# vadimkantorov/convasr

Hardware: NVIDIA B200
Metric: audio_seconds_per_second (higher is better)
Workload: dtype bf16

## Files before the change

### convasr_b200/csrc/common.cuh

```cuda
#pragma once
#include <cuda_runtime.h>
#include <cuda_bf16.h>
#include <cuda_fp16.h>
#include <cuda.h>
#include <stdint.h>
#include <math.h>

namespace cab {

void set_last_error(const char* fmt, ...);

#define CAB_CHECK_ARG(cond, ...)                                  \
    do {                                                          \
        if (!(cond)) {                                            \
            ::cab::set_last_error(__VA_ARGS__);                   \
            return -1;                                            \
        }                                                         \
    } while (0)

#define CAB_CHECK_CUDA(expr)                                                              \
    do {                                                                                  \
        cudaError_t _e = (expr);                                                          \
        if (_e != cudaSuccess) {                                                          \
            ::cab::set_last_error("%s failed: %s (%s:%d)", #expr, cudaGetErrorString(_e), \
// ... 81 lines not shown
        : "=r"(ok)
        : "r"(smem_u32(bar)), "r"(parity)
        : "memory");
    return ok != 0;
}
#ifndef CAB_MBAR_SPIN_LIMIT
#define CAB_MBAR_SPIN_LIMIT (1u << 28)
#endif
__device__ __forceinline__ void mbar_wait(uint64_t* bar, uint32_t parity) {
    uint32_t spins = 0;
    while (!mbar_try_wait(bar, parity)) {
        if (++spins > CAB_MBAR_SPIN_LIMIT) __trap();
    }
}

__device__ __forceinline__ void tma_prefetch_desc(const CUtensorMap* m) {
    asm volatile("prefetch.tensormap [%0];" ::"l"(reinterpret_cast<uint64_t>(m)) : "memory");
}
__device__ __forceinline__ void tma_load_3d(void* smem_dst, const CUtensorMap* m, uint64_t* bar,
                                            int c0, int c1, int c2) {
    asm volatile(
        "cp.async.bulk.tensor.3d.shared::cluster.global.tile.mbarrier::complete_tx::bytes "
        "[%0], [%1, {%3, %4, %5}], [%2];"
        ::"r"(smem_u32(smem_dst)), "l"(reinterpret_cast<uint64_t>(m)), "r"(smem_u32(bar)),
        "r"(c0), "r"(c1), "r"(c2)
        : "memory");
}

__device__ __forceinline__ void tma_load_4d(void* smem_dst, const CUtensorMap* m, uint64_t* bar,
                                            int c0, int c1, int c2, int c3) {
// ... 32 lines not shown
        "setp.ne.b32 p, %4, 0;\n\t"
        "tcgen05.mma.cta_group::1.kind::f16 [%0], %1, %2, %3, p;\n\t"
        "}\n"
        ::"r"(tmem_d), "l"(desc_a), "l"(desc_b), "r"(idesc), "r"(accumulate)
        : "memory");
}
__device__ __forceinline__ void umma_e4m3(uint32_t tmem_d, uint64_t desc_a, uint64_t desc_b,
                                          uint32_t idesc, uint32_t accumulate) {
    asm volatile(
        "{\n\t"
        ".reg .pred p;\n\t"
        "setp.ne.b32 p, %4, 0;\n\t"
        "tcgen05.mma.cta_group::1.kind::f8f6f4 [%0], %1, %2, %3, p;\n\t"
        "}\n"
        ::"r"(tmem_d), "l"(desc_a), "l"(desc_b), "r"(idesc), "r"(accumulate)
        : "memory");
}
__device__ __forceinline__ void umma_commit(uint64_t* bar) {
    asm volatile("tcgen05.commit.cta_group::1.mbarrier::arrive::one.shared::cluster.b64 [%0];" ::"r"(
                     smem_u32(bar))
                 : "memory");
}
__device__ __forceinline__ void tmem_ld_32x32(uint32_t taddr, uint32_t (&v)[32]) {
    asm volatile(
        "tcgen05.ld.sync.aligned.32x32b.x32.b32 "
        "{%0, %1, %2, %3, %4, %5, %6, %7, %8, %9, %10, %11, %12, %13, %14, %15, "
        "%16, %17, %18, %19, %20, %21, %22, %23, %24, %25, %26, %27, %28, %29, %30, %31}, [%32];"
        : "=r"(v[0]), "=r"(v[1]), "=r"(v[2]), "=r"(v[3]), "=r"(v[4]), "=r"(v[5]), "=r"(v[6]),
          "=r"(v[7]), "=r"(v[8]), "=r"(v[9]), "=r"(v[10]), "=r"(v[11]), "=r"(v[12]), "=r"(v[13]),
          "=r"(v[14]), "=r"(v[15]), "=r"(v[16]), "=r"(v[17]), "=r"(v[18]), "=r"(v[19]),
// ... 53 lines not shown
```

### convasr_b200/csrc/conv_gemm.cu

```cuda
#include "common.cuh"
#include "../../include/convasr_b200.h"
#include <mutex>
#include <atomic>

namespace cab {

constexpr int kBlockM = 128;
constexpr int kBlockK = 64;
constexpr int kStages = 4;
constexpr int kMaxBlockN = 256;
constexpr int kATileBytes = kBlockM * kBlockK * 2;
constexpr int kBTileBytes = kMaxBlockN * kBlockK * 2;
constexpr int kStageBytes = kATileBytes + kBTileBytes;
constexpr int kAccStages = 2;
constexpr int kTmemCols = 512;
constexpr int kNumThreads = 256;
constexpr int kEpiCols = 32;
constexpr int kEpiTileBytes = kBlockM * kEpiCols * 2;
constexpr int kOffStageOut = kStages * kStageBytes;
constexpr int kOffBias = kOffStageOut + 4 * kEpiTileBytes;
constexpr int kOffBars = kOffBias + kMaxBlockN * 4;
constexpr int kSmemBytes = kOffBars + 1024  + 256 ;
static_assert(kSmemBytes <= 232448, "exceeds the 227 KB dynamic shared memory limit");

struct SrcDev {
    int a_ch_off, w_ch_off, n_chunks, taps, dil, pad_left;
};

struct alignas(64) ConvParams {
    CUtensorMap amap[CAB_MAX_CONV_SOURCES];
    CUtensorMap wmap[CAB_MAX_CONV_SOURCES];
    CUtensorMap omap_hi, omap_lo;
    SrcDev src[CAB_MAX_CONV_SOURCES];
    int n_src;
    int B, T_out, C_out, block_n;
    int mtiles_per_b, n_ntiles, n_tiles;
    int epilogue, act;
    float act_a, act_b;
    const float* bias;
    const float* xlen;
    __nv_bfloat16* out_hi;
    __nv_bfloat16* out_lo;
    int out_T_rows, out_ld;
    float* logits;
    float* log_probs;
    int* argmax;
    double* stats;
    float* lse;
    int mtile_major;
    const float* skip_frac;
    int skip_T, skip_margin;
// ... 3 lines not shown
    double* bnr_partials;
    int bnr_C, bnr_act;
    float bnr_a, bnr_b;
    const float* alpha;
    float out_inv;
};

__device__ __forceinline__ int live_mtiles(const ConvParams& p, int b) {
    if (p.skip_frac == nullptr) return p.mtiles_per_b;
    const int rows = min(p.T_out, frac_len(__ldg(p.skip_frac + b), p.skip_T) + p.skip_margin);
    return rows <= 0 ? 0 : (rows + 127) / 128;
}
#define CAB_NEXT_UNIT()                                                        \
    int am, nt;                                                                \
    if (p.mtile_major) {                                                       \
        if (nt_next == 0) u += gridDim.x;                                      \
        am = u;                                                                \
        nt = nt_next;                                                          \
        nt_next = nt_next + 1 == p.n_ntiles ? 0 : nt_next + 1;                 \
    } else {                                                                   \
        u += gridDim.x;                                                        \
        nt = u % p.n_ntiles;                                                   \
        am = u / p.n_ntiles;                                                   \
    }
struct TileCursor {
    int b, base, end;
    __device__ __forceinline__ void init(const ConvParams& p) { b = 0; base = 0; end = live_mtiles(p, 0); }
    __device__ __forceinline__ bool seek(const ConvParams& p, int am) {
        while (am >= end) {
            if (++b >= p.B) return false;
            base = end;
            end += live_mtiles(p, b);
        }
        return true;
    }
};

__device__ __forceinline__ float apply_act(float x, int act, float a, float b) {
    switch (act) {
        case CAB_ACT_RELU: return fmaxf(x, 0.f);
        case CAB_ACT_HARDTANH: return fminf(fmaxf(x, a), b);
        case CAB_ACT_LEAKY_RELU: return x > 0.f ? x : x * a;
        default: return x;
    }
}

__device__ __forceinline__ void tma_store_3d(const CUtensorMap* m, const void* smem_src, int c0, int c1, int c2) {
    asm volatile("cp.async.bulk.tensor.3d.global.shared::cta.bulk_group [%0, {%2, %3, %4}], [%1];" ::"l"(
                     reinterpret_cast<uint64_t>(m)),
                 "r"(smem_u32(smem_src)), "r"(c0), "r"(c1), "r"(c2)
// ... 92 lines not shown
    const int cq = c >> 3, cb = (c & 7) << 1;
    float s = 0.f, q = 0.f;
#pragma unroll 8
    for (int r = rg * 32; r < r_end; ++r) {
        const int off = r * 64 + ((cq ^ ((r >> 1) & 3)) << 4) + cb;
        float x = __uint_as_float((uint32_t)(*reinterpret_cast<const uint16_t*>(st_h + off)) << 16);
        if (LO) x += __uint_as_float((uint32_t)(*reinterpret_cast<const uint16_t*>(st_l + off)) << 16);
        s += x;
        q = fmaf(x, x, q);
    }
    s_out = s;
    q_out = q;
}

template <bool FP8>
__global__ void __launch_bounds__(kNumThreads, 1)
conv1d_umma_kernel(const __grid_constant__ ConvParams p) {
    constexpr int kChunk = FP8 ? 2 * kBlockK : kBlockK;
    extern __shared__ uint8_t smem_raw[];
    uint8_t* smem = reinterpret_cast<uint8_t*>((reinterpret_cast<uintptr_t>(smem_raw) + 1023) &
                                               ~uintptr_t(1023));
    uint64_t* full_bar = reinterpret_cast<uint64_t*>(smem + kOffBars);
    float* s_bias = reinterpret_cast<float*>(smem + kOffBias);
    uint64_t* empty_bar = full_bar + kStages;
    uint64_t* tmem_full = empty_bar + kStages;
    uint64_t* tmem_empty = tmem_full + kAccStages;
    uint32_t* tmem_ptr = reinterpret_cast<uint32_t*>(tmem_empty + kAccStages);
    uint64_t* ybar = tmem_empty + kAccStages + 1;

    const int warp = threadIdx.x >> 5;
    const int lane = threadIdx.x & 31;

    if (warp == 0 && lane == 0) {
        for (int s = 0; s < p.n_src; ++s) {
            tma_prefetch_desc(&p.amap[s]);
            tma_prefetch_desc(&p.wmap[s]);
        }
        if (p.epilogue == CAB_EPI_LOGITS_ROWS) tma_prefetch_desc(&p.omap_hi);
        if (p.epilogue == CAB_EPI_ACT_BF16) {
            tma_prefetch_desc(&p.omap_hi);
            if (p.out_lo != nullptr) tma_prefetch_desc(&p.omap_lo);
            if (p.bnr_partials != nullptr) tma_prefetch_desc(&p.ymap);
        }
    }
    if (warp == 1 && lane == 0) {
        for (int i = 0; i < kStages; ++i) {
            mbar_init(&full_bar[i], 1);
            mbar_init(&empty_bar[i], 1);
        }
        for (int i = 0; i < kAccStages; ++i) {
            mbar_init(&tmem_full[i], 1);
            mbar_init(&tmem_empty[i], 4);
        }
        mbar_init(&ybar[0], 1);
        mbar_init(&ybar[1], 1);
        mbar_fence_init();
    }
    if (warp == 2) {
        tmem_alloc(tmem_ptr, kTmemCols);
        tmem_relinquish();
    }
    tc_fence_before();
    __syncthreads();
    tc_fence_after();
    const uint32_t tmem_base = *tmem_ptr;

    const int block_n = p.block_n;
    const uint32_t stage_tx_bytes = kATileBytes + block_n * kBlockK * 2;

    if (warp == 0) {
        if (lane == 0) {
            int stage = 0;
            uint32_t phase = 0;
            TileCursor cur;
            cur.init(p);
            int u = (int)blockIdx.x - (int)gridDim.x, nt_next = 0;
            for (;;) {
                CAB_NEXT_UNIT()
                if (!cur.seek(p, am)) break;
                const int b = cur.b;
                const int t0 = (am - cur.base) * kBlockM;
                const int n0 = nt * block_n;
                for (int s = 0; s < p.n_src; ++s) {
                    const SrcDev sd = p.src[s];
                    for (int tap = 0; tap < sd.taps; ++tap) {
                        const int trow = t0 + tap * sd.dil - sd.pad_left;
                        for (int ch = 0; ch < sd.n_chunks; ++ch) {
                            mbar_wait(&empty_bar[stage], phase ^ 1);
                            uint8_t* a_dst = smem + stage * kStageBytes;
                            uint8_t* b_dst = a_dst + kATileBytes;
                            mbar_expect_tx(&full_bar[stage], stage_tx_bytes);
                            tma_load_3d(a_dst, &p.amap[s], &full_bar[stage],
                                        sd.a_ch_off + ch * kChunk, trow, b);
                            tma_load_3d(b_dst, &p.wmap[s], &full_bar[stage],
                                        sd.w_ch_off + ch * kChunk, n0, tap);
                            if (++stage == kStages) { stage = 0; phase ^= 1; }
                        }
                    }
                }
            }
        }
    } else if (warp == 1) {
        if (lane == 0) {
            const uint32_t idesc = FP8 ? umma_idesc_e4m3(kBlockM, block_n) : umma_idesc_bf16(kBlockM, block_n);
            int stage = 0;
            uint32_t phase = 0;
            int acc = 0;
            uint32_t acc_phase = 0;
            TileCursor cur;
            cur.init(p);
            int u = (int)blockIdx.x - (int)gridDim.x, nt_next = 0;
            for (;;) {
                CAB_NEXT_UNIT()
                (void)nt;
                if (!cur.seek(p, am)) break;
                mbar_wait(&tmem_empty[acc], acc_phase ^ 1);
                tc_fence_after();
                const uint32_t d_tmem = tmem_base + acc * kMaxBlockN;
                uint32_t accumulate = 0;
                for (int s = 0; s < p.n_src; ++s) {
                    const int ksteps = p.src[s].taps * p.src[s].n_chunks;
                    for (int ks = 0; ks < ksteps; ++ks) {
                        mbar_wait(&full_bar[stage], phase);
                        tc_fence_after();
                        const uint32_t a_addr = smem_u32(smem + stage * kStageBytes);
                        const uint32_t b_addr = a_addr + kATileBytes;
                        const uint64_t a_desc = umma_desc_sw128(a_addr);
                        const uint64_t b_desc = umma_desc_sw128(b_addr);
#pragma unroll
                        for (int k = 0; k < kBlockK / 16; ++k) {
                            if (FP8) umma_e4m3(d_tmem, a_desc + 2 * k, b_desc + 2 * k, idesc, accumulate);
                            else umma_bf16(d_tmem, a_desc + 2 * k, b_desc + 2 * k, idesc, accumulate);
                            accumulate = 1;
                        }
                        umma_commit(&empty_bar[stage]);
                        if (++stage == kStages) { stage = 0; phase ^= 1; }
                    }
                }
                umma_commit(&tmem_full[acc]);
                if (++acc == kAccStages) { acc = 0; acc_phase ^= 1; }
            }
        }
    } else if (warp >= 4) {
        const int q = warp & 3;
        const int row = q * 32 + lane;
        int acc = 0;
        uint32_t acc_phase = 0;
        uint32_t epi_chunks = 0;
        TileCursor cur;
        cur.init(p);
        float run_m = -INFINITY, run_s = 0.f;
        int run_i = 0;
        uint32_t yphase = 0;
        const bool fold = p.bnr_partials != nullptr;
        int u = (int)blockIdx.x - (int)gridDim.x, nt_next = 0;
        for (;;) {
            CAB_NEXT_UNIT()
            if (!cur.seek(p, am)) break;
            const int b = cur.b;
            const int t0 = (am - cur.base) * kBlockM;
            const int n0 = nt * block_n;
            const int t = t0 + row;
            const bool row_ok = t < p.T_out;

            const uint32_t taddr = tmem_base + acc * kMaxBlockN + (uint32_t(q * 32) << 16);
            if (p.epilogue != CAB_EPI_ACT_BF16) {
                mbar_wait(&tmem_full[acc], acc_phase);
                tc_fence_after();
            }

            if (p.epilogue == CAB_EPI_ACT_BF16) {
                int len = p.T_out;
                if (p.xlen != nullptr) len = frac_len(__ldg(p.xlen + b), p.T_out);
                const bool keep = t < len;
                const int et = threadIdx.x - 128;
                const bool has_lo = p.out_lo != nullptr;
                uint8_t* const ystage = smem + kOffStageOut + 2 * kEpiTileBytes;
                int bnr_rows = 0;
                if (fold) {
                    if (et == 0) {
                        const int ybuf = epi_chunks & 1;
                        mbar_expect_tx(&ybar[ybuf], kEpiTileBytes);
                        tma_load_3d(ystage + ybuf * kEpiTileBytes, &p.ymap, &ybar[ybuf], n0, t0, b);
                    }
                    int blen = p.T_out;
                    if (p.bnr_xlen != nullptr) blen = min(blen, frac_len(__ldg(p.bnr_xlen + b), p.T_out));
                    bnr_rows = min(max(blen - t0, 0), kBlockM);
                }
                epi_bar(1);
                float* const s_alpha = reinterpret_cast<float*>(smem + kOffStageOut + 2 * kEpiTileBytes);
                for (int i = et; i < block_n; i += 128) {
                    const int n = n0 + i;
                    s_bias[i] = (p.bias != nullptr && n < p.C_out) ? __ldg(p.bias + n) : 0.f;
                    if (FP8) s_alpha[i] = n < p.C_out ? __ldg(p.alpha + n) : 0.f;
                }
                epi_bar(1);
                mbar_wait(&tmem_full[acc], acc_phase);
                tc_fence_after();
                uint8_t* stage = smem + kOffStageOut;
                for (int c0 = 0; c0 < block_n; c0 += kEpiCols) {
                    if (n0 + c0 >= p.C_out) break;
                    uint32_t v[32];
                    tmem_ld_32x32(taddr + c0, v);
                    tmem_ld_wait();
                    if (c0 + kEpiCols >= block_n || n0 + c0 + kEpiCols >= p.C_out) {
                        tc_fence_before();
                        __syncwarp();
                        if (lane == 0) mbar_arrive(&tmem_empty[acc]);
                    }
                    const int buf = epi_chunks & 1;
                    uint8_t* st_hi = stage + buf * kEpiTileBytes;
                    uint8_t* st_lo = stage + (2 + buf) * kEpiTileBytes;
                    if (et == 0) bulk_wait_read<1>();
                    float bnr_sc = 0.f, bnr_sh = 0.f;
                    const int bnr_col = n0 + c0 + (et & 31);
                    if (fold && bnr_col < p.bnr_C) {
                        bnr_sc = __ldg(p.bnr_ss + bnr_col);
                        bnr_sh = __ldg(p.bnr_ss + p.bnr_C + bnr_col);
                    }
                    epi_bar(2);
                    if (fold && et == 0 && c0 + kEpiCols < block_n && n0 + c0 + kEpiCols < p.C_out) {
                        const int ynext = (epi_chunks + 1) & 1;
                        mbar_expect_tx(&ybar[ynext], kEpiTileBytes);
// ... 2 lines not shown
                    const float* sb = s_bias + c0;
#define CAB_EPI_CALL(ACT)                                                                          \
    if (FP8) epi_chunk_e4m3<ACT>(v, sb, s_alpha + c0, p.act_a, p.act_b, keep, p.out_inv, row, st_hi); \
    else if (has_lo) epi_chunk<ACT, true>(v, sb, p.act_a, p.act_b, keep, row, st_hi, st_lo);       \
    else epi_chunk<ACT, false>(v, sb, p.act_a, p.act_b, keep, row, st_hi, st_lo);
                    switch (p.act) {
                        case CAB_ACT_RELU: CAB_EPI_CALL(CAB_ACT_RELU) break;
                        case CAB_ACT_HARDTANH: CAB_EPI_CALL(CAB_ACT_HARDTANH) break;
                        case CAB_ACT_LEAKY_RELU: CAB_EPI_CALL(CAB_ACT_LEAKY_RELU) break;
                        default: CAB_EPI_CALL(CAB_ACT_NONE) break;
                    }
#undef CAB_EPI_CALL
                    fence_async_smem();
                    epi_bar(3);
                    if (et == 0) {
                        tma_store_3d(&p.omap_hi, st_hi, n0 + c0, t0, b);
                        if (has_lo) tma_store_3d(&p.omap_lo, st_lo, n0 + c0, t0, b);
                        bulk_commit();
                    }
                    if (p.stats != nullptr) {
                        float cs, cq;
                        const int srows = min(max(p.T_out - t0, 0), kBlockM);
                        if (has_lo) stats_column_pass<true>(st_hi, st_lo, et, srows, cs, cq);
                        else stats_column_pass<false>(st_hi, st_lo, et, srows, cs, cq);
                        const int col = n0 + c0 + (et & 31);
                        if (col < p.C_out && srows > (et >> 5) * 32) {
                            atomicAdd(p.stats + col, (double)cs);
                            atomicAdd(p.stats + p.C_out + col, (double)cq);
                        }
                    }
                    if (fold) {
                        mbar_wait(&ybar[buf], (yphase >> buf) & 1u);
                        yphase ^= 1u << buf;
                        const uint8_t* st_y = ystage + buf * kEpiTileBytes;
                        float cs, cq;
                        switch (p.bnr_act) {
                            case CAB_ACT_RELU: bnr_column_pass<CAB_ACT_RELU>(st_hi, st_y, et, bnr_rows, bnr_sc, bnr_sh, p.bnr_a, p.bnr_b, cs, cq); break;
// ... 18 lines not shown
                for (int i = et; i < block_n; i += 128) {
                    const int n = n0 + i;
                    s_bias[i] = (p.bias != nullptr && n < C) ? __ldg(p.bias + n) : 0.f;
                }
                epi_bar(1);
                if (nt == 0) { run_m = -INFINITY; run_s = 0.f; run_i = 0; }
                uint8_t* stage = smem + kOffStageOut;
                for (int c0 = 0; c0 < block_n; c0 += 32) {
                    if (n0 + c0 >= C) break;
                    uint32_t v[32];
                    tmem_ld_32x32(taddr + c0, v);
                    tmem_ld_wait();
                    if (c0 + 32 >= block_n || n0 + c0 + 32 >= C) {
                        tc_fence_before();
                        __syncwarp();
                        if (lane == 0) mbar_arrive(&tmem_empty[acc]);
                    }
                    float x[32];
                    float cm = -INFINITY;
                    int ci = 0;
#pragma unroll
                    for (int j = 0; j < 32; ++j) {
                        const bool in = n0 + c0 + j < C;
                        if (FP8) x[j] = fmaf(__uint_as_float(v[j]), in ? __ldg(p.alpha + n0 + c0 + j) : 0.f, s_bias[c0 + j]);
                        else x[j] = __uint_as_float(v[j]) + s_bias[c0 + j];
                        if (in && x[j] > cm) { cm = x[j]; ci = n0 + c0 + j; }
                    }
                    if (cm > run_m) {
                        run_s *= __expf(run_m - cm);
                        run_m = cm;
                        run_i = ci;
                    }
                    float cs = 0.f;
#pragma unroll
                    for (int j = 0; j < 32; ++j) cs += (n0 + c0 + j < C) ? __expf(x[j] - run_m) : 0.f;
                    run_s += cs;
                    const int buf = epi_chunks & 1;
                    uint8_t* st = stage + buf * (2 * kEpiTileBytes);
                    if (et == 0) bulk_wait_read<1>();
                    epi_bar(2);
#pragma unroll
                    for (int q4 = 0; q4 < 8; ++q4)
                        *reinterpret_cast<float4*>(st + row * 128 + ((q4 ^ (row & 7)) << 4)) = make_float4(x[4 * q4], x[4 * q4 + 1], x[4 * q4 + 2], x[4 * q4 + 3]);
                    fence_async_smem();
                    epi_bar(3);
                    if (et == 0) {
                        tma_store_3d(&p.omap_hi, st, n0 + c0, t0, b);
                        bulk_commit();
                    }
                    ++epi_chunks;
                }
                if (nt == p.n_ntiles - 1 && row_ok) {
                    if (p.lse) p.lse[size_t(b) * p.T_out + t] = run_m + logf(run_s);
                    if (p.argmax) p.argmax[size_t(b) * p.T_out + t] = run_i;
                }
                if (++acc == kAccStages) { acc = 0; acc_phase ^= 1; }
                continue;
            } else if (p.epilogue == CAB_EPI_LOGSOFTMAX) {
                const int C = p.C_out;
                float vmax = -INFINITY;
                int imax = 0;
                for (int c0 = 0; c0 < C; c0 += 16) {
// ... 50 lines not shown
                    tmem_ld_wait();
                    if (row_ok) {
#pragma unroll
                        for (int j = 0; j < 16; ++j) {
                            const int c = n0 + c0 + j;
                            if (c < C) {
                                float x = (FP8 ? __uint_as_float(v[j]) * __ldg(p.alpha + c) : __uint_as_float(v[j])) + (p.bias ? __ldg(p.bias + c) : 0.f);
                                p.logits[(size_t(b) * C + c) * p.T_out + t] = apply_act(x, p.act, p.act_a, p.act_b);
                            }
                        }
                    }
                }
            }
            tc_fence_before();
            __syncwarp();
            if (lane == 0) mbar_arrive(&tmem_empty[acc]);
            if (++acc == kAccStages) { acc = 0; acc_phase ^= 1; }
        }
        if (p.skip_frac != nullptr && p.epilogue == CAB_EPI_ACT_BF16) {
            const int et = threadIdx.x - 128;
            const bool has_lo = p.out_lo != nullptr;
            uint8_t* stage = smem + kOffStageOut;
            int b = 0, base = 0, end = p.mtiles_per_b - live_mtiles(p, 0);
            for (int z = blockIdx.x;; z += gridDim.x) {
                const int nt = z % p.n_ntiles;
                const int sm = z / p.n_ntiles;
                bool done = false;
                while (sm >= end) {
                    if (++b >= p.B) { done = true; break; }
                    base = end;
                    end += p.mtiles_per_b - live_mtiles(p, b);
                }
                if (done) break;
                const int t0 = (live_mtiles(p, b) + (sm - base)) * kBlockM;
                const int n0 = nt * block_n;
                for (int c0 = 0; c0 < block_n; c0 += kEpiCols) {
                    if (n0 + c0 >= p.C_out) break;
                    const int buf = epi_chunks & 1;
                    uint8_t* st_hi = stage + buf * kEpiTileBytes;
                    uint8_t* st_lo = stage + (2 + buf) * kEpiTileBytes;
                    if (et == 0) bulk_wait_read<1>();
                    epi_bar(2);
                    uint4* zh = reinterpret_cast<uint4*>(st_hi + row * (FP8 ? 32 : 64));
                    uint4* zl = reinterpret_cast<uint4*>(st_lo + row * 64);
#pragma unroll
                    for (int qd = 0; qd < (FP8 ? 2 : 4); ++qd) {
                        zh[qd] = make_uint4(0, 0, 0, 0);
                        if (has_lo) zl[qd] = make_uint4(0, 0, 0, 0);
                    }
                    fence_async_smem();
                    epi_bar(3);
                    if (et == 0) {
                        tma_store_3d(&p.omap_hi, st_hi, n0 + c0, t0, b);
                        if (has_lo) tma_store_3d(&p.omap_lo, st_lo, n0 + c0, t0, b);
                        bulk_commit();
                    }
                    ++epi_chunks;
                }
            }
        }
        if (threadIdx.x == 128) bulk_wait_all();
    }

    tc_fence_before();
    __syncthreads();
    if (warp == 2) {
        tc_fence_after();
        tmem_dealloc(tmem_base, kTmemCols);
    }
}

typedef CUresult (*EncodeTiledFn)(CUtensorMap*, CUtensorMapDataType, cuuint32_t, void*,
                                  const cuuint64_t*, const cuuint64_t*, const cuuint32_t*,
                                  const cuuint32_t*, CUtensorMapInterleave, CUtensorMapSwizzle,
                                  CUtensorMapL2promotion, CUtensorMapFloatOOBfill);

static EncodeTiledFn get_encode_fn() {
    static EncodeTiledFn fn = nullptr;
    static std::once_flag once;
    std::call_once(once, [] {
        void* ptr = nullptr;
        cudaDriverEntryPointQueryResult qres;
        if (cudaGetDriverEntryPoint("cuTensorMapEncodeTiled", &ptr, cudaEnableDefault, &qres) ==
// ... 14 lines not shown
    cuuint32_t box[3] = {box0, box1, 1};
    cuuint32_t estr[3] = {1, 1, 1};
    CUresult r = enc(map, elem_bytes == 1 ? CU_TENSOR_MAP_DATA_TYPE_UINT8 : CU_TENSOR_MAP_DATA_TYPE_BFLOAT16, 3, const_cast<void*>(base), dims,
                     strides, box, estr, CU_TENSOR_MAP_INTERLEAVE_NONE,
                     swizzle, CU_TENSOR_MAP_L2_PROMOTION_L2_256B,
                     CU_TENSOR_MAP_FLOAT_OOB_FILL_NONE);
    CAB_CHECK_ARG(r == CUDA_SUCCESS,
                  "cuTensorMapEncodeTiled failed (%d): base=%p dims=%llu,%llu,%llu pitch=%llu,%llu "
                  "box=%u,%u",
                  (int)r, base, (unsigned long long)d0, (unsigned long long)d1,
                  (unsigned long long)d2, (unsigned long long)pitch1_elems,
                  (unsigned long long)pitch2_elems, box0, box1);
    return 0;
}

static int pick_block_n(int C_out, int epilogue, long long m_tiles, int num_sms) {
    if (epilogue == CAB_EPI_LOGSOFTMAX) return ((C_out + 15) / 16) * 16;
    int best_bn = 0;
    double best_cost = 0.0;
    const int min_tiles = (C_out + kMaxBlockN - 1) / kMaxBlockN;
    for (int n_tiles = min_tiles; n_tiles <= min_tiles * 8; ++n_tiles) {
        int bn = (C_out + n_tiles - 1) / n_tiles;
        bn = ((bn + 31) / 32) * 32;
        if (bn < 64 && n_tiles > min_tiles) break;
        const long long tiles = m_tiles * ((C_out + bn - 1) / bn);
        const double cost = (double)((tiles + num_sms - 1) / num_sms) * (bn + 96);
        if (best_bn == 0 || cost < best_cost * 0.98) { best_bn = bn; best_cost = cost; }
    }
    return best_bn;
}

extern std::atomic<int64_t> g_launch_count;

}

using namespace cab;

template <bool FP8>
static int conv1d_launch(const cab_conv_source_t* srcs, int n_src, const cab_conv_epilogue_t* ep, const float* alpha,
                         float out_inv, cudaStream_t stream) {
    constexpr int kChunk = FP8 ? 2 * kBlockK : kBlockK;
    constexpr int kElem = FP8 ? 1 : 2;
    CAB_CHECK_ARG(srcs && ep, "null sources/epilogue");
    CAB_CHECK_ARG(n_src >= 1 && n_src <= CAB_MAX_CONV_SOURCES, "n_sources=%d out of [1,%d]", n_src,
                  CAB_MAX_CONV_SOURCES);
    CAB_CHECK_ARG(ep->B > 0 && ep->T_out > 0 && ep->C_out > 0, "bad output shape B=%d T=%d C=%d",
                  ep->B, ep->T_out, ep->C_out);

    static thread_local ConvParams p;
    p.n_src = n_src;
    p.B = ep->B;
    p.T_out = ep->T_out;
    p.C_out = ep->C_out;
    static int sms_for_tiling = 0;
    if (sms_for_tiling == 0) {
        int dev = 0;
        cudaGetDevice(&dev);
        cudaDeviceGetAttribute(&sms_for_tiling, cudaDevAttrMultiProcessorCount, dev);
        if (sms_for_tiling <= 0) sms_for_tiling = 148;
    }
    int bn = ep->block_n > 0 ? ep->block_n : pick_block_n(ep->C_out, ep->epilogue, (long long)ep->B * ((ep->T_out + kBlockM - 1) / kBlockM), sms_for_tiling);
    CAB_CHECK_ARG(bn % 16 == 0 && bn >= 16 && bn <= kMaxBlockN, "block_n=%d must be a multiple of 16 in [16,256]", bn);
    if (ep->epilogue == CAB_EPI_ACT_BF16) {
        CAB_CHECK_ARG(bn % 32 == 0, "block_n=%d must be a multiple of 32 for the bf16 epilogue", bn);
        CAB_CHECK_ARG(ep->C_out % 32 == 0, "C_out=%d must be a multiple of 32 (pad on the host)", ep->C_out);
        CAB_CHECK_ARG(ep->out_hi != nullptr, "out_hi is null");
        CAB_CHECK_ARG(ep->out_ld_ch >= ep->C_out && ep->out_ld_ch % 8 == 0, "bad out_ld_ch=%d", ep->out_ld_ch);
        CAB_CHECK_ARG(ep->out_T_rows >= ep->T_out, "out_T_rows=%d < T_out=%d", ep->out_T_rows, ep->T_out);
        CAB_CHECK_ARG((reinterpret_cast<uintptr_t>(ep->out_hi) & 15) == 0, "out_hi must be 16-byte aligned");
    } else if (ep->epilogue == CAB_EPI_LOGSOFTMAX) {
        CAB_CHECK_ARG(ep->C_out <= kMaxBlockN, "log_softmax epilogue supports at most %d classes (got %d)", kMaxBlockN, ep->C_out);
        CAB_CHECK_ARG(bn >= ep->C_out, "block_n=%d must cover all %d classes", bn, ep->C_out);
    } else if (ep->epilogue == CAB_EPI_LOGITS_F32) {
        CAB_CHECK_ARG(ep->logits != nullptr, "logits is null");
    } else if (ep->epilogue == CAB_EPI_LOGITS_ROWS) {
        CAB_CHECK_ARG(ep->logits != nullptr, "logits is null");
        CAB_CHECK_ARG(bn % 32 == 0, "block_n=%d must be a multiple of 32 for the row-major logits epilogue", bn);
        CAB_CHECK_ARG(ep->out_ld_ch >= ep->C_out && ep->out_ld_ch % 4 == 0 && (reinterpret_cast<uintptr_t>(ep->logits) & 15) == 0, "row-major logits need a 16-byte aligned base and a row pitch that is a multiple of 4 floats (got %d)", ep->out_ld_ch);
        CAB_CHECK_ARG(ep->act == CAB_ACT_NONE, "the row-major logits epilogue applies no activation");
    } else {
        CAB_CHECK_ARG(false, "unknown epilogue %d", ep->epilogue);
    }
    p.block_n = bn;
    p.mtiles_per_b = (ep->T_out + kBlockM - 1) / kBlockM;
    p.n_ntiles = (ep->C_out + bn - 1) / bn;
    p.n_tiles = p.B * p.mtiles_per_b * p.n_ntiles;
    p.epilogue = ep->epilogue;
    p.act = ep->act;
    p.act_a = ep->act_a;
    p.act_b = ep->act_b;
    p.bias = ep->bias;
    p.xlen = ep->xlen_frac;
    p.out_hi = static_cast<__nv_bfloat16*>(ep->out_hi);
    p.out_lo = static_cast<__nv_bfloat16*>(ep->out_lo);
    p.out_T_rows = ep->out_T_rows;
    p.out_ld = ep->out_ld_ch;
    p.logits = ep->logits;
    p.log_probs = ep->log_probs;
    p.argmax = ep->argmax;
    p.stats = ep->epilogue == CAB_EPI_ACT_BF16 ? ep->stats : nullptr;
    p.lse = ep->epilogue == CAB_EPI_LOGITS_ROWS ? ep->log_probs : nullptr;
// ... 56 lines not shown
    }

    for (int s = 0; s < n_src; ++s) {
        const cab_conv_source_t& c = srcs[s];
        CAB_CHECK_ARG(c.act && c.wgt, "source %d: null pointer", s);
        CAB_CHECK_ARG(c.C_in > 0 && c.C_in % kChunk == 0, "source %d: C_in=%d must be a multiple of %d", s, c.C_in, kChunk);
        CAB_CHECK_ARG(c.ch_off >= 0 && c.ch_off + c.C_in <= c.ld_ch && c.ld_ch % (16 / kElem) == 0, "source %d: bad channel window off=%d C_in=%d ld=%d", s, c.ch_off, c.C_in, c.ld_ch);
        CAB_CHECK_ARG(c.w_ch_off >= 0 && c.w_ch_off + c.C_in <= c.w_ld_ch && c.w_ld_ch % (16 / kElem) == 0, "source %d: bad weight channel window", s);
        CAB_CHECK_ARG(c.taps >= 1 && c.dilation >= 1, "source %d: taps=%d dilation=%d", s, c.taps, c.dilation);
        CAB_CHECK_ARG(c.T_in >= 1 && c.T_rows >= c.T_in, "source %d: T_in=%d T_rows=%d", s, c.T_in, c.T_rows);
        CAB_CHECK_ARG((reinterpret_cast<uintptr_t>(c.act) & 15) == 0 && (reinterpret_cast<uintptr_t>(c.wgt) & 15) == 0, "source %d: pointers must be 16-byte aligned", s);
        int rc = encode_map_3d(&p.amap[s], c.act, (uint64_t)c.ld_ch, (uint64_t)c.T_in, (uint64_t)ep->B,
                               (uint64_t)c.ld_ch, (uint64_t)c.T_rows * c.ld_ch, kChunk, kBlockM, CU_TENSOR_MAP_SWIZZLE_128B, kElem);
        if (rc) return rc;
        rc = encode_map_3d(&p.wmap[s], c.wgt, (uint64_t)c.w_ld_ch, (uint64_t)c.w_rows, (uint64_t)c.taps,
                           (uint64_t)c.w_ld_ch, (uint64_t)c.w_rows * c.w_ld_ch, kChunk, (uint32_t)bn, CU_TENSOR_MAP_SWIZZLE_128B, kElem);
        if (rc) return rc;
        p.src[s].a_ch_off = c.ch_off;
        p.src[s].w_ch_off = c.w_ch_off;
        p.src[s].n_chunks = c.C_in / kChunk;
        p.src[s].taps = c.taps;
        p.src[s].dil = c.dilation;
        p.src[s].pad_left = c.pad_left;
    }

    static int num_sms = 0;
    static std::once_flag once;
    static cudaError_t attr_err = cudaSuccess;
    std::call_once(once, [] {
        int dev = 0;
        cudaGetDevice(&dev);
        cudaDeviceGetAttribute(&num_sms, cudaDevAttrMultiProcessorCount, dev);
        attr_err = cudaFuncSetAttribute(conv1d_umma_kernel<FP8>, cudaFuncAttributeMaxDynamicSharedMemorySize, kSmemBytes);
    });
    CAB_CHECK_ARG(attr_err == cudaSuccess, "cudaFuncSetAttribute(smem=%d) failed: %s", kSmemBytes, cudaGetErrorString(attr_err));
    CAB_CHECK_ARG(num_sms > 0, "no CUDA device");
    int grid = p.n_tiles < num_sms ? p.n_tiles : num_sms;
    if (p.mtile_major) grid = p.B * p.mtiles_per_b < num_sms ? p.B * p.mtiles_per_b : num_sms;
    conv1d_umma_kernel<FP8><<<grid, kNumThreads, kSmemBytes, stream>>>(p);
    CAB_CHECK_LAUNCH();
    g_launch_count.fetch_add(1, std::memory_order_relaxed);
    return 0;
}

extern "C" int cab_conv1d_fused(const cab_conv_source_t* srcs, int n_src,
                                const cab_conv_epilogue_t* ep, cab_stream_t stream) {
    return conv1d_launch<false>(srcs, n_src, ep, nullptr, 1.f, static_cast<cudaStream_t>(stream));
}

extern "C" int cab_conv1d_fused_fp8(const cab_conv_source_t* srcs, int n_src, const cab_conv_epilogue_t* ep,
                                    const float* alpha, float out_scale_inv, cab_stream_t stream) {
    return conv1d_launch<true>(srcs, n_src, ep, alpha, out_scale_inv, static_cast<cudaStream_t>(stream));
}
// ... 1 lines not shown
```

### convasr_b200/csrc/ctc.cu

```cuda
#include "common.cuh"
#include "../../include/convasr_b200.h"
#include <atomic>
#include <float.h>
#include <cuda_fp16.h>

namespace cab {
extern std::atomic<int64_t> g_launch_count;

constexpr int kCtcMaxPer = 4;

__device__ __forceinline__ float lse3(float a, float b, float c) {
    const float m = fmaxf(a, fmaxf(b, c));
    if (m == -INFINITY) return -INFINITY;
    return logf(expf(a - m) + expf(b - m) + expf(c - m)) + m;
}
__device__ __forceinline__ float lse2(float a, float b) {
    const float m = fmaxf(a, b);
    if (m == -INFINITY) return -INFINITY;
    return logf(expf(a - m) + expf(b - m)) + m;
}

constexpr int kCtcPrefetch = 8;

__device__ __forceinline__ float lse3_fast(float a, float b, float c) {
// ... 366 lines not shown
            if (t > 0) {
                s -= (int)bp[(size_t)t * S_max + s];
                if (s < 0) s = 0;
            }
        }
    }
}

constexpr int kAlignClusterMax = 16;
constexpr int kAlignGroupsPer = 2;
constexpr int kAlignCtaStates = 4 * kAlignGroupsPer * 1024;
constexpr int kAlignLongMaxL = (kAlignClusterMax * kAlignCtaStates - 1) / 2;

__device__ __forceinline__ void cluster_arrive() { asm volatile("barrier.cluster.arrive.release.aligned;" ::: "memory"); }
__device__ __forceinline__ void cluster_wait() { asm volatile("barrier.cluster.wait.acquire.aligned;" ::: "memory"); }
__device__ __forceinline__ uint32_t cluster_ctarank() {
    uint32_t r;
    asm volatile("mov.u32 %0, %%cluster_ctarank;" : "=r"(r));
    return r;
}
__device__ __forceinline__ uint32_t cluster_nctarank() {
    uint32_t r;
    asm volatile("mov.u32 %0, %%cluster_nctarank;" : "=r"(r));
    return r;
}
__device__ __forceinline__ float* cluster_map(float* p, uint32_t rank) {
    uint64_t out;
    asm volatile("mapa.u64 %0, %1, %2;" : "=l"(out) : "l"(reinterpret_cast<uint64_t>(p)), "r"(rank));
    return reinterpret_cast<float*>(out);
}

template <bool HALF>
__global__ void __launch_bounds__(1024, 1)
ctc_align_cluster_kernel(const float* __restrict__ lp, int64_t st, int64_t sb, int64_t sc, const int64_t* __restrict__ targets,
                         const int64_t* __restrict__ in_len, const int64_t* __restrict__ tgt_len, int T, int L_max, int blank,
// ... 1019 lines not shown
```

Baseline: 52400.

## Run conv GEMM as 2-CTA cluster pairs with cta_group::2 UMMA

Converts the conv1d UMMA kernel to 2-CTA clusters. Each pair computes a 256-row M tile with tcgen05 cta_group::2 MMA, and each CTA loads half the B (weight) tile, which halves weight smem traffic per CTA and lets the pipeline grow from 4 to 6 stages. Tile scheduling, TMEM alloc and dealloc, and barriers are reworked for cluster-wide arrivals, and grid sizing uses occupancy-derived max clusters. Odd M tile counts leave a half-idle CTA, and the cross-CTA synchronisation adds complexity and deadlock risk.

```diff
diff --git a/convasr_b200/csrc/common.cuh b/convasr_b200/csrc/common.cuh
--- a/convasr_b200/csrc/common.cuh
+++ b/convasr_b200/csrc/common.cuh
@@ -119,6 +119,32 @@
     }
 }
 
+__device__ __forceinline__ uint32_t cluster_ctarank() {
+    uint32_t r;
+    asm volatile("mov.u32 %0, %%cluster_ctarank;" : "=r"(r));
+    return r;
+}
+__device__ __forceinline__ void cluster_sync() {
+    asm volatile("barrier.cluster.arrive.release.aligned;\n\tbarrier.cluster.wait.acquire.aligned;" ::: "memory");
+}
+__device__ __forceinline__ uint32_t mapa_shared(const void* p, uint32_t rank) {
+    uint32_t r;
+    asm volatile("mapa.shared::cluster.u32 %0, %1, %2;" : "=r"(r) : "r"(smem_u32(p)), "r"(rank));
+    return r;
+}
+__device__ __forceinline__ void mbar_arrive_cluster(uint32_t cluster_addr) {
+    asm volatile("mbarrier.arrive.release.cluster.shared::cluster.b64 _, [%0];" ::"r"(cluster_addr) : "memory");
+}
+
+__device__ __forceinline__ void tma_load_3d_pair(void* smem_dst, const CUtensorMap* m, uint32_t bar_cluster_addr,
+                                                 int c0, int c1, int c2) {
+    asm volatile(
+        "cp.async.bulk.tensor.3d.cta_group::2.shared::cluster.global.tile.mbarrier::complete_tx::bytes "
+        "[%0], [%1, {%3, %4, %5}], [%2];"
+        ::"r"(smem_u32(smem_dst)), "l"(reinterpret_cast<uint64_t>(m)), "r"(bar_cluster_addr),
+        "r"(c0), "r"(c1), "r"(c2)
+        : "memory");
+}
 __device__ __forceinline__ void tma_prefetch_desc(const CUtensorMap* m) {
     asm volatile("prefetch.tensormap [%0];" ::"l"(reinterpret_cast<uint64_t>(m)) : "memory");
 }
@@ -181,6 +207,43 @@
         "tcgen05.mma.cta_group::1.kind::f8f6f4 [%0], %1, %2, %3, p;\n\t"
         "}\n"
         ::"r"(tmem_d), "l"(desc_a), "l"(desc_b), "r"(idesc), "r"(accumulate)
+        : "memory");
+}
+__device__ __forceinline__ void tmem_alloc_pair(uint32_t* smem_dst, uint32_t ncols) {
+    asm volatile("tcgen05.alloc.cta_group::2.sync.aligned.shared::cta.b32 [%0], %1;" ::"r"(smem_u32(smem_dst)), "r"(ncols)
+                 : "memory");
+}
+__device__ __forceinline__ void tmem_relinquish_pair() {
+    asm volatile("tcgen05.relinquish_alloc_permit.cta_group::2.sync.aligned;" ::: "memory");
+}
+__device__ __forceinline__ void tmem_dealloc_pair(uint32_t taddr, uint32_t ncols) {
+    asm volatile("tcgen05.dealloc.cta_group::2.sync.aligned.b32 %0, %1;" ::"r"(taddr), "r"(ncols) : "memory");
+}
+template <bool FP8>
+__device__ __forceinline__ void umma_pair(uint32_t tmem_d, uint64_t desc_a, uint64_t desc_b, uint32_t idesc, uint32_t accumulate) {
+    if (FP8)
+        asm volatile(
+            "{\n\t"
+            ".reg .pred p;\n\t"
+            "setp.ne.b32 p, %4, 0;\n\t"
+            "tcgen05.mma.cta_group::2.kind::f8f6f4 [%0], %1, %2, %3, p;\n\t"
+            "}\n"
+            ::"r"(tmem_d), "l"(desc_a), "l"(desc_b), "r"(idesc), "r"(accumulate)
+            : "memory");
+    else
+        asm volatile(
+            "{\n\t"
+            ".reg .pred p;\n\t"
+            "setp.ne.b32 p, %4, 0;\n\t"
+            "tcgen05.mma.cta_group::2.kind::f16 [%0], %1, %2, %3, p;\n\t"
+            "}\n"
+            ::"r"(tmem_d), "l"(desc_a), "l"(desc_b), "r"(idesc), "r"(accumulate)
+            : "memory");
+}
+__device__ __forceinline__ void umma_commit_pair(uint64_t* bar) {
+    asm volatile(
+        "tcgen05.commit.cta_group::2.mbarrier::arrive::one.shared::cluster.multicast::cluster.b64 [%0], %1;" ::"r"(smem_u32(bar)),
+        "h"((uint16_t)0x3)
         : "memory");
 }
 __device__ __forceinline__ void umma_commit(uint64_t* bar) {
diff --git a/convasr_b200/csrc/conv_gemm.cu b/convasr_b200/csrc/conv_gemm.cu
--- a/convasr_b200/csrc/conv_gemm.cu
+++ b/convasr_b200/csrc/conv_gemm.cu
@@ -7,10 +7,10 @@
 
 constexpr int kBlockM = 128;
 constexpr int kBlockK = 64;
-constexpr int kStages = 4;
+constexpr int kStages = 6;
 constexpr int kMaxBlockN = 256;
 constexpr int kATileBytes = kBlockM * kBlockK * 2;
-constexpr int kBTileBytes = kMaxBlockN * kBlockK * 2;
+constexpr int kBTileBytes = kMaxBlockN / 2 * kBlockK * 2;
 constexpr int kStageBytes = kATileBytes + kBTileBytes;
 constexpr int kAccStages = 2;
 constexpr int kTmemCols = 512;
@@ -34,7 +34,7 @@
     SrcDev src[CAB_MAX_CONV_SOURCES];
     int n_src;
     int B, T_out, C_out, block_n;
-    int mtiles_per_b, n_ntiles, n_tiles;
+    int mtiles_per_b, n_ntiles;
     int epilogue, act;
     float act_a, act_b;
     const float* bias;
@@ -68,26 +68,29 @@
 #define CAB_NEXT_UNIT()                                                        \
     int am, nt;                                                                \
     if (p.mtile_major) {                                                       \
-        if (nt_next == 0) u += gridDim.x;                                      \
+        if (nt_next == 0) u += nclusters;                                      \
         am = u;                                                                \
         nt = nt_next;                                                          \
         nt_next = nt_next + 1 == p.n_ntiles ? 0 : nt_next + 1;                 \
     } else {                                                                   \
-        u += gridDim.x;                                                        \
+        u += nclusters;                                                        \
         nt = u % p.n_ntiles;                                                   \
         am = u / p.n_ntiles;                                                   \
     }
 struct TileCursor {
-    int b, base, end;
-    __device__ __forceinline__ void init(const ConvParams& p) { b = 0; base = 0; end = live_mtiles(p, 0); }
+    int b, base, end, live;
+    __device__ __forceinline__ void init(const ConvParams& p) { b = 0; base = 0; live = live_mtiles(p, 0); end = (live + 1) >> 1; }
     __device__ __forceinline__ bool seek(const ConvParams& p, int am) {
         while (am >= end) {
             if (++b >= p.B) return false;
             base = end;
-            end += live_mtiles(p, b);
+            live = live_mtiles(p, b);
+            end += (live + 1) >> 1;
         }
         return true;
     }
+    __device__ __forceinline__ int t0(int am, uint32_t rank) const { return ((am - base) * 2 + (int)rank) * kBlockM; }
+    __device__ __forceinline__ bool half_live(int am, uint32_t rank) const { return (am - base) * 2 + (int)rank < live; }
 };
 
 __device__ __forceinline__ float apply_act(float x, int act, float a, float b) {
@@ -210,7 +213,7 @@
 }
 
 template <bool FP8>
-__global__ void __launch_bounds__(kNumThreads, 1)
+__global__ void __cluster_dims__(2, 1, 1) __launch_bounds__(kNumThreads, 1)
 conv1d_umma_kernel(const __grid_constant__ ConvParams p) {
     constexpr int kChunk = FP8 ? 2 * kBlockK : kBlockK;
     extern __shared__ uint8_t smem_raw[];
@@ -226,6 +229,8 @@
 
     const int warp = threadIdx.x >> 5;
     const int lane = threadIdx.x & 31;
+    const uint32_t rank = cluster_ctarank();
+    const int cluster = (int)blockIdx.x >> 1, nclusters = (int)gridDim.x >> 1;
 
     if (warp == 0 && lane == 0) {
         for (int s = 0; s < p.n_src; ++s) {
@@ -246,23 +251,22 @@
         }
         for (int i = 0; i < kAccStages; ++i) {
             mbar_init(&tmem_full[i], 1);
-            mbar_init(&tmem_empty[i], 4);
+            mbar_init(&tmem_empty[i], 8);
         }
         mbar_init(&ybar[0], 1);
         mbar_init(&ybar[1], 1);
         mbar_fence_init();
     }
     if (warp == 2) {
-        tmem_alloc(tmem_ptr, kTmemCols);
-        tmem_relinquish();
+        tmem_alloc_pair(tmem_ptr, kTmemCols);
+        tmem_relinquish_pair();
     }
     tc_fence_before();
-    __syncthreads();
+    cluster_sync();
     tc_fence_after();
     const uint32_t tmem_base = *tmem_ptr;
 
     const int block_n = p.block_n;
-    const uint32_t stage_tx_bytes = kATileBytes + block_n * kBlockK * 2;
 
     if (warp == 0) {
         if (lane == 0) {
@@ -270,13 +274,15 @@
             uint32_t phase = 0;
             TileCursor cur;
             cur.init(p);
-            int u = (int)blockIdx.x - (int)gridDim.x, nt_next = 0;
+            int u = cluster - nclusters, nt_next = 0;
+            const uint32_t full0 = mapa_shared(full_bar, 0);
+            const uint32_t pair_tx_bytes = 2 * kATileBytes + block_n * kBlockK * 2;
             for (;;) {
                 CAB_NEXT_UNIT()
                 if (!cur.seek(p, am)) break;
                 const int b = cur.b;
-                const int t0 = (am - cur.base) * kBlockM;
-                const int n0 = nt * block_n;
+                const int t0 = cur.t0(am, rank);
+                const int n0 = nt * block_n + (int)rank * (block_n >> 1);
                 for (int s = 0; s < p.n_src; ++s) {
                     const SrcDev sd = p.src[s];
                     for (int tap = 0; tap < sd.taps; ++tap) {
@@ -285,27 +291,30 @@
                             mbar_wait(&empty_bar[stage], phase ^ 1);
                             uint8_t* a_dst = smem + stage * kStageBytes;
                             uint8_t* b_dst = a_dst + kATileBytes;
-                            mbar_expect_tx(&full_bar[stage], stage_tx_bytes);
-                            tma_load_3d(a_dst, &p.amap[s], &full_bar[stage],
-                                        sd.a_ch_off + ch * kChunk, trow, b);
-                            tma_load_3d(b_dst, &p.wmap[s], &full_bar[stage],
-                                        sd.w_ch_off + ch * kChunk, n0, tap);
+                            if (rank == 0) mbar_expect_tx(&full_bar[stage], pair_tx_bytes);
+                            const uint32_t fb = full0 + stage * 8;
+                            tma_load_3d_pair(a_dst, &p.amap[s], fb, sd.a_ch_off + ch * kChunk, trow, b);
+                            tma_load_3d_pair(b_dst, &p.wmap[s], fb, sd.w_ch_off + ch * kChunk, n0, tap);
                             if (++stage == kStages) { stage = 0; phase ^= 1; }
                         }
                     }
                 }
             }
+            for (int i = 0; i < kStages; ++i) {
+                mbar_wait(&empty_bar[stage], phase ^ 1);
+                if (++stage == kStages) { stage = 0; phase ^= 1; }
+            }
         }
     } else if (warp == 1) {
-        if (lane == 0) {
-            const uint32_t idesc = FP8 ? umma_idesc_e4m3(kBlockM, block_n) : umma_idesc_bf16(kBlockM, block_n);
+        if (lane == 0 && rank == 0) {
+            const uint32_t idesc = FP8 ? umma_idesc_e4m3(2 * kBlockM, block_n) : umma_idesc_bf16(2 * kBlockM, block_n);
             int stage = 0;
             uint32_t phase = 0;
             int acc = 0;
             uint32_t acc_phase = 0;
             TileCursor cur;
             cur.init(p);
-            int u = (int)blockIdx.x - (int)gridDim.x, nt_next = 0;
+            int u = cluster - nclusters, nt_next = 0;
             for (;;) {
                 CAB_NEXT_UNIT()
                 (void)nt;
@@ -325,15 +334,14 @@
                         const uint64_t b_desc = umma_desc_sw128(b_addr);
 #pragma unroll
                         for (int k = 0; k < kBlockK / 16; ++k) {
-                            if (FP8) umma_e4m3(d_tmem, a_desc + 2 * k, b_desc + 2 * k, idesc, accumulate);
-                            else umma_bf16(d_tmem, a_desc + 2 * k, b_desc + 2 * k, idesc, accumulate);
+                            umma_pair<FP8>(d_tmem, a_desc + 2 * k, b_desc + 2 * k, idesc, accumulate);
                             accumulate = 1;
                         }
-                        umma_commit(&empty_bar[stage]);
+                        umma_commit_pair(&empty_bar[stage]);
                         if (++stage == kStages) { stage = 0; phase ^= 1; }
                     }
                 }
-                umma_commit(&tmem_full[acc]);
+                umma_commit_pair(&tmem_full[acc]);
                 if (++acc == kAccStages) { acc = 0; acc_phase ^= 1; }
             }
         }
@@ -349,12 +357,14 @@
         int run_i = 0;
         uint32_t yphase = 0;
         const bool fold = p.bnr_partials != nullptr;
-        int u = (int)blockIdx.x - (int)gridDim.x, nt_next = 0;
+        const uint32_t tmem_empty0 = mapa_shared(tmem_empty, 0);
+        int u = cluster - nclusters, nt_next = 0;
         for (;;) {
             CAB_NEXT_UNIT()
             if (!cur.seek(p, am)) break;
             const int b = cur.b;
-            const int t0 = (am - cur.base) * kBlockM;
+            const int t0 = cur.t0(am, rank);
+            const bool live = cur.half_live(am, rank);
             const int n0 = nt * block_n;
             const int t = t0 + row;
             const bool row_ok = t < p.T_out;
@@ -368,7 +378,7 @@
             if (p.epilogue == CAB_EPI_ACT_BF16) {
                 int len = p.T_out;
                 if (p.xlen != nullptr) len = frac_len(__ldg(p.xlen + b), p.T_out);
-                const bool keep = t < len;
+                const bool keep = t < len && live;
                 const int et = threadIdx.x - 128;
                 const bool has_lo = p.out_lo != nullptr;
                 uint8_t* const ystage = smem + kOffStageOut + 2 * kEpiTileBytes;
@@ -381,7 +391,7 @@
                     }
                     int blen = p.T_out;
                     if (p.bnr_xlen != nullptr) blen = min(blen, frac_len(__ldg(p.bnr_xlen + b), p.T_out));
-                    bnr_rows = min(max(blen - t0, 0), kBlockM);
+                    bnr_rows = live ? min(max(blen - t0, 0), kBlockM) : 0;
                 }
                 epi_bar(1);
                 float* const s_alpha = reinterpret_cast<float*>(smem + kOffStageOut + 2 * kEpiTileBytes);
@@ -402,7 +412,7 @@
                     if (c0 + kEpiCols >= block_n || n0 + c0 + kEpiCols >= p.C_out) {
                         tc_fence_before();
                         __syncwarp();
-                        if (lane == 0) mbar_arrive(&tmem_empty[acc]);
+                        if (lane == 0) mbar_arrive_cluster(tmem_empty0 + acc * 8);
                     }
                     const int buf = epi_chunks & 1;
                     uint8_t* st_hi = stage + buf * kEpiTileBytes;
@@ -435,13 +445,15 @@
                     fence_async_smem();
                     epi_bar(3);
                     if (et == 0) {
-                        tma_store_3d(&p.omap_hi, st_hi, n0 + c0, t0, b);
-                        if (has_lo) tma_store_3d(&p.omap_lo, st_lo, n0 + c0, t0, b);
+                        if (t0 < p.T_out) {
+                            tma_store_3d(&p.omap_hi, st_hi, n0 + c0, t0, b);
+                            if (has_lo) tma_store_3d(&p.omap_lo, st_lo, n0 + c0, t0, b);
+                        }
                         bulk_commit();
                     }
                     if (p.stats != nullptr) {
                         float cs, cq;
-                        const int srows = min(max(p.T_out - t0, 0), kBlockM);
+                        const int srows = live ? min(max(p.T_out - t0, 0), kBlockM) : 0;
                         if (has_lo) stats_column_pass<true>(st_hi, st_lo, et, srows, cs, cq);
                         else stats_column_pass<false>(st_hi, st_lo, et, srows, cs, cq);
                         const int col = n0 + c0 + (et & 31);
@@ -490,7 +502,7 @@
                     if (c0 + 32 >= block_n || n0 + c0 + 32 >= C) {
                         tc_fence_before();
                         __syncwarp();
-                        if (lane == 0) mbar_arrive(&tmem_empty[acc]);
+                        if (lane == 0) mbar_arrive_cluster(tmem_empty0 + acc * 8);
                     }
                     float x[32];
                     float cm = -INFINITY;
@@ -521,7 +533,7 @@
                     fence_async_smem();
                     epi_bar(3);
                     if (et == 0) {
-                        tma_store_3d(&p.omap_hi, st, n0 + c0, t0, b);
+                        if (t0 < p.T_out) tma_store_3d(&p.omap_hi, st, n0 + c0, t0, b);
                         bulk_commit();
                     }
                     ++epi_chunks;
@@ -602,14 +614,15 @@
             }
             tc_fence_before();
             __syncwarp();
-            if (lane == 0) mbar_arrive(&tmem_empty[acc]);
+            if (lane == 0) mbar_arrive_cluster(tmem_empty0 + acc * 8);
             if (++acc == kAccStages) { acc = 0; acc_phase ^= 1; }
         }
         if (p.skip_frac != nullptr && p.epilogue == CAB_EPI_ACT_BF16) {
             const int et = threadIdx.x - 128;
             const bool has_lo = p.out_lo != nullptr;
             uint8_t* stage = smem + kOffStageOut;
-            int b = 0, base = 0, end = p.mtiles_per_b - live_mtiles(p, 0);
+            auto covered = [&](int bb) { return min(p.mtiles_per_b, (live_mtiles(p, bb) + 1) & ~1); };
+            int b = 0, base = 0, end = p.mtiles_per_b - covered(0);
             for (int z = blockIdx.x;; z += gridDim.x) {
                 const int nt = z % p.n_ntiles;
                 const int sm = z / p.n_ntiles;
@@ -617,10 +630,10 @@
                 while (sm >= end) {
                     if (++b >= p.B) { done = true; break; }
                     base = end;
-                    end += p.mtiles_per_b - live_mtiles(p, b);
+                    end += p.mtiles_per_b - covered(b);
                 }
                 if (done) break;
-                const int t0 = (live_mtiles(p, b) + (sm - base)) * kBlockM;
+                const int t0 = (covered(b) + (sm - base)) * kBlockM;
                 const int n0 = nt * block_n;
                 for (int c0 = 0; c0 < block_n; c0 += kEpiCols) {
                     if (n0 + c0 >= p.C_out) break;
@@ -651,10 +664,10 @@
     }
 
     tc_fence_before();
-    __syncthreads();
+    cluster_sync();
     if (warp == 2) {
         tc_fence_after();
-        tmem_dealloc(tmem_base, kTmemCols);
+        tmem_dealloc_pair(tmem_base, kTmemCols);
     }
 }
 
@@ -699,7 +712,7 @@
     return 0;
 }
 
-static int pick_block_n(int C_out, int epilogue, long long m_tiles, int num_sms) {
+static int pick_block_n(int C_out, int epilogue, long long m_pairs, int num_pairs) {
     if (epilogue == CAB_EPI_LOGSOFTMAX) return ((C_out + 15) / 16) * 16;
     int best_bn = 0;
     double best_cost = 0.0;
@@ -708,8 +721,8 @@
         int bn = (C_out + n_tiles - 1) / n_tiles;
         bn = ((bn + 31) / 32) * 32;
         if (bn < 64 && n_tiles > min_tiles) break;
-        const long long tiles = m_tiles * ((C_out + bn - 1) / bn);
-        const double cost = (double)((tiles + num_sms - 1) / num_sms) * (bn + 96);
+        const long long units = m_pairs * ((C_out + bn - 1) / bn);
+        const double cost = (double)((units + num_pairs - 1) / num_pairs) * (bn + 96);
         if (best_bn == 0 || cost < best_cost * 0.98) { best_bn = bn; best_cost = cost; }
     }
     return best_bn;
@@ -737,14 +750,25 @@
     p.B = ep->B;
     p.T_out = ep->T_out;
     p.C_out = ep->C_out;
-    static int sms_for_tiling = 0;
-    if (sms_for_tiling == 0) {
-        int dev = 0;
+    static int max_pairs = 0;
+    static std::once_flag once;
+    static cudaError_t attr_err = cudaSuccess;
+    std::call_once(once, [] {
+        attr_err = cudaFuncSetAttribute(conv1d_umma_kernel<FP8>, cudaFuncAttributeMaxDynamicSharedMemorySize, kSmemBytes);
+        if (attr_err != cudaSuccess) return;
+        int dev = 0, sms = 0;
         cudaGetDevice(&dev);
-        cudaDeviceGetAttribute(&sms_for_tiling, cudaDevAttrMultiProcessorCount, dev);
-        if (sms_for_tiling <= 0) sms_for_tiling = 148;
-    }
-    int bn = ep->block_n > 0 ? ep->block_n : pick_block_n(ep->C_out, ep->epilogue, (long long)ep->B * ((ep->T_out + kBlockM - 1) / kBlockM), sms_for_tiling);
+        cudaDeviceGetAttribute(&sms, cudaDevAttrMultiProcessorCount, dev);
+        cudaLaunchConfig_t cfg = {};
+        cfg.gridDim = dim3((unsigned)(sms & ~1));
+        cfg.blockDim = dim3(kNumThreads);
+        cfg.dynamicSmemBytes = kSmemBytes;
+        attr_err = cudaOccupancyMaxActiveClusters(&max_pairs, conv1d_umma_kernel<FP8>, &cfg);
+    });
+    CAB_CHECK_ARG(attr_err == cudaSuccess, "conv kernel set-up (smem=%d, CTA pairs) failed: %s", kSmemBytes, cudaGetErrorString(attr_err));
+    CAB_CHECK_ARG(max_pairs > 0, "no CUDA device, or no CTA pair of the conv kernel fits on it");
+    const long long m_pairs = (long long)ep->B * (((ep->T_out + kBlockM - 1) / kBlockM + 1) / 2);
+    int bn = ep->block_n > 0 ? ep->block_n : pick_block_n(ep->C_out, ep->epilogue, m_pairs, max_pairs);
     CAB_CHECK_ARG(bn % 16 == 0 && bn >= 16 && bn <= kMaxBlockN, "block_n=%d must be a multiple of 16 in [16,256]", bn);
     if (ep->epilogue == CAB_EPI_ACT_BF16) {
         CAB_CHECK_ARG(bn % 32 == 0, "block_n=%d must be a multiple of 32 for the bf16 epilogue", bn);
@@ -769,7 +793,6 @@
     p.block_n = bn;
     p.mtiles_per_b = (ep->T_out + kBlockM - 1) / kBlockM;
     p.n_ntiles = (ep->C_out + bn - 1) / bn;
-    p.n_tiles = p.B * p.mtiles_per_b * p.n_ntiles;
     p.epilogue = ep->epilogue;
     p.act = ep->act;
     p.act_a = ep->act_a;
@@ -856,7 +879,7 @@
                                (uint64_t)c.ld_ch, (uint64_t)c.T_rows * c.ld_ch, kChunk, kBlockM, CU_TENSOR_MAP_SWIZZLE_128B, kElem);
         if (rc) return rc;
         rc = encode_map_3d(&p.wmap[s], c.wgt, (uint64_t)c.w_ld_ch, (uint64_t)c.w_rows, (uint64_t)c.taps,
-                           (uint64_t)c.w_ld_ch, (uint64_t)c.w_rows * c.w_ld_ch, kChunk, (uint32_t)bn, CU_TENSOR_MAP_SWIZZLE_128B, kElem);
+                           (uint64_t)c.w_ld_ch, (uint64_t)c.w_rows * c.w_ld_ch, kChunk, (uint32_t)bn / 2, CU_TENSOR_MAP_SWIZZLE_128B, kElem);
         if (rc) return rc;
         p.src[s].a_ch_off = c.ch_off;
         p.src[s].w_ch_off = c.w_ch_off;
@@ -866,19 +889,8 @@
         p.src[s].pad_left = c.pad_left;
     }
 
-    static int num_sms = 0;
-    static std::once_flag once;
-    static cudaError_t attr_err = cudaSuccess;
-    std::call_once(once, [] {
-        int dev = 0;
-        cudaGetDevice(&dev);
-        cudaDeviceGetAttribute(&num_sms, cudaDevAttrMultiProcessorCount, dev);
-        attr_err = cudaFuncSetAttribute(conv1d_umma_kernel<FP8>, cudaFuncAttributeMaxDynamicSharedMemorySize, kSmemBytes);
-    });
-    CAB_CHECK_ARG(attr_err == cudaSuccess, "cudaFuncSetAttribute(smem=%d) failed: %s", kSmemBytes, cudaGetErrorString(attr_err));
-    CAB_CHECK_ARG(num_sms > 0, "no CUDA device");
-    int grid = p.n_tiles < num_sms ? p.n_tiles : num_sms;
-    if (p.mtile_major) grid = p.B * p.mtiles_per_b < num_sms ? p.B * p.mtiles_per_b : num_sms;
+    const long long units = p.mtile_major ? m_pairs : m_pairs * p.n_ntiles;
+    const int grid = 2 * (int)(units < max_pairs ? units : max_pairs);
     conv1d_umma_kernel<FP8><<<grid, kNumThreads, kSmemBytes, stream>>>(p);
     CAB_CHECK_LAUNCH();
     g_launch_count.fetch_add(1, std::memory_order_relaxed);
diff --git a/convasr_b200/csrc/ctc.cu b/convasr_b200/csrc/ctc.cu
--- a/convasr_b200/csrc/ctc.cu
+++ b/convasr_b200/csrc/ctc.cu
@@ -404,11 +404,6 @@
 
 __device__ __forceinline__ void cluster_arrive() { asm volatile("barrier.cluster.arrive.release.aligned;" ::: "memory"); }
 __device__ __forceinline__ void cluster_wait() { asm volatile("barrier.cluster.wait.acquire.aligned;" ::: "memory"); }
-__device__ __forceinline__ uint32_t cluster_ctarank() {
-    uint32_t r;
-    asm volatile("mov.u32 %0, %%cluster_ctarank;" : "=r"(r));
-    return r;
-}
 __device__ __forceinline__ uint32_t cluster_nctarank() {
     uint32_t r;
     asm volatile("mov.u32 %0, %%cluster_nctarank;" : "=r"(r));
```

After: 53880, median of 6. 2.8% higher.
